# Sreyan88/audio-ssl

Hardware: AMD Instinct MI355X
Metric: upstream clips/sec (1s@16kHz, 64-mel) (higher is better)
Workload: dtype bf16; 1 GPU; delores-m upstream step (log-mel + 2 views + q/k conv encoders + MoCo + 3 Barlow heads + bwd + SGD), 1 s @ 16 kHz, 64 mel, batch 512/GPU, queue 65536; global_batch=512, parallelism=dp1

## Files before the change

### audio-ssl_amd/csrc/conv1.hip

```cpp
#include <cstdlib>
#include "common.h"

namespace {

constexpr int NTAP = 9, NMOM = 9 + 45;
constexpr int MOM_REPL = 16;

__device__ __forceinline__ int tri(int a, int b) {
    return a * 9 - a * (a - 1) / 2 + (b - a);
}

constexpr int MOM_TC = 128;
__global__ __launch_bounds__(256) void conv1_moments_kernel(const float* __restrict__ img, double* __restrict__ mom,
                                                            int N, int F, int T, int nchunk, int tcw) {
    extern __shared__ float tile[];
    __shared__ float sh[4][NMOM];
    const int n = blockIdx.x / nchunk, t0 = (blockIdx.x - n * nchunk) * tcw;
    const int tc = min(tcw, T - t0), ld = tc + 2;
    const float* im = img + (long)n * F * T;
    {
        const int total = (F + 2) * ld, dr = 256 / ld, dc = 256 - dr * ld;
        int r = threadIdx.x / ld, cidx = threadIdx.x - r * ld;
        for (int i0 = threadIdx.x; i0 < total; i0 += 8 * 256) {
            float v[8];
            int rr = r, cc = cidx;
#pragma unroll
            for (int k = 0; k < 8; ++k) {
                const int f = rr - 1, t = t0 + cc - 1;
                v[k] = (i0 + k * 256 < total && f >= 0 && f < F && t >= 0 && t < T) ? im[f * T + t] : 0.f;
                cc += dc; rr += dr;
                if (cc >= ld) { cc -= ld; ++rr; }
            }
#pragma unroll
            for (int k = 0; k < 8; ++k)
                if (i0 + k * 256 < total) tile[i0 + k * 256] = v[k];
            r = rr; cidx = cc;
        }
    }
    __syncthreads();
    float acc[NMOM];
#pragma unroll
    for (int i = 0; i < NMOM; ++i) acc[i] = 0.f;
    const int df = 256 / tc, dt = 256 - df * tc;
    int f = threadIdx.x / tc, t = threadIdx.x - f * tc;
    for (; f < F;) {
        const float* c = tile + f * ld + t;
        float x[NTAP];
#pragma unroll
        for (int kh = 0; kh < 3; ++kh)
#pragma unroll
            for (int kw = 0; kw < 3; ++kw) x[kh * 3 + kw] = c[kh * ld + kw];
#pragma unroll
        for (int a = 0; a < 9; ++a) {
            acc[a] += x[a];
#pragma unroll
            for (int b = 0; b < 9; ++b)
                if (b >= a) acc[9 + tri(a, b)] += x[a] * x[b];
        }
        t += dt; f += df;
        if (t >= tc) { t -= tc; ++f; }
    }
    const int lane = threadIdx.x & 63, w = threadIdx.x >> 6;
#pragma unroll
    for (int i = 0; i < NMOM; ++i) {
        const float v = wave_sum(acc[i]);
        if (lane == 0) sh[w][i] = v;
    }
    __syncthreads();
    if (threadIdx.x < NMOM) {
        const double v = (double)sh[0][threadIdx.x] + (double)sh[1][threadIdx.x] + (double)sh[2][threadIdx.x] +
                         (double)sh[3][threadIdx.x];
        atomicAdd(&mom[(blockIdx.x & (MOM_REPL - 1)) * NMOM + threadIdx.x], v);
    }
}

__global__ __launch_bounds__(576) void conv1_finalize_kernel(double* __restrict__ momr, const float* __restrict__ w,
                                      const float* __restrict__ bias, const float* __restrict__ gamma,
                                      const float* __restrict__ beta, float* running_mean, float* running_var,
                                      float momentum, float eps, double count, float* scale, float* shift,
                                      float* save_mean, float* save_rstd, int repl) {
    __shared__ double tot[NMOM];
    __shared__ double cov[81];
    __shared__ double rowv[64][9], rowm[64][9];
    const int i = threadIdx.x;
    if (i < NMOM) {
        double t = 0.0;
        for (int r = 0; r < repl; ++r) t += momr[r * NMOM + i];
        tot[i] = t;
    }
    __syncthreads();
    if (i < NMOM) momr[i] = tot[i];
    if (i < 81) {
        const int a = i / 9, bb = i - a * 9;
        const double s2 = tot[9 + (a <= bb ? tri(a, bb) : tri(bb, a))] / count;
        cov[i] = s2 - (tot[a] / count) * (tot[bb] / count);
    }
    __syncthreads();
    const int c = i / 9, a = i - (i / 9) * 9;
    if (i < 576) {
        double r = 0.0;
        for (int bb = 0; bb < 9; ++bb) r += (double)w[c * 9 + bb] * cov[a * 9 + bb];
        rowv[c][a] = (double)w[c * 9 + a] * r;
        rowm[c][a] = (double)w[c * 9 + a] * tot[a];
    }
    __syncthreads();
    if (i < 576 && a == 0) {
        double mean = 0.0, var = 0.0;
        for (int k = 0; k < 9; ++k) { mean += rowm[c][k]; var += rowv[c][k]; }
        mean = mean / count;
        var = var < 0.0 ? 0.0 : var;
        mean += (double)bias[c];
        const double rstd = 1.0 / sqrt(var + (double)eps);
        const float sc = (float)((double)gamma[c] * rstd);
        scale[c] = sc;
        shift[c] = (float)((double)beta[c] - mean * (double)gamma[c] * rstd);
        save_mean[c] = (float)mean;
        save_rstd[c] = (float)rstd;
        if (running_mean) {
            running_mean[c] = (1.f - momentum) * running_mean[c] + momentum * (float)mean;
            running_var[c] = (1.f - momentum) * running_var[c] + momentum * (float)(var * count / (count - 1.0));
        }
    }
}

__device__ __forceinline__ void load_patch(float* patch, const float* __restrict__ img, int n, int tp, int F, int T) {
    const float* im = img + (long)n * F * T;
    for (int i = threadIdx.x; i < (F + 2) * 4; i += 256) {
        const int f = (i >> 2) - 1, t = 2 * tp - 1 + (i & 3);
        patch[i] = (f >= 0 && f < F && t >= 0 && t < T) ? im[f * T + t] : 0.f;
    }
}

struct PatchRegs {
    float v[2];
    __device__ __forceinline__ void fetch(const float* __restrict__ img, int n, int tp, int F, int T) {
        const float* im = img + (long)n * F * T;
#pragma unroll
        for (int j = 0; j < 2; ++j) {
            const int i = threadIdx.x + j * 256;
            const int f = (i >> 2) - 1, t = 2 * tp - 1 + (i & 3);
            v[j] = (i < (F + 2) * 4 && f >= 0 && f < F && t >= 0 && t < T) ? im[f * T + t] : 0.f;
        }
    }
    __device__ __forceinline__ void put(float* patch, int F) const {
#pragma unroll
// ... 135 lines not shown
__device__ __forceinline__ Vec8<bf16> stem_taps(const float* patch, int f, int dt, int half) {
    Vec8<bf16> a;
    if (half == 0) {
        a.v[0] = (bf16)patch[(f + 0) * 4 + dt + 0]; a.v[1] = (bf16)patch[(f + 0) * 4 + dt + 1]; a.v[2] = (bf16)patch[(f + 0) * 4 + dt + 2];
        a.v[3] = (bf16)patch[(f + 1) * 4 + dt + 0]; a.v[4] = (bf16)patch[(f + 1) * 4 + dt + 1]; a.v[5] = (bf16)patch[(f + 1) * 4 + dt + 2];
        a.v[6] = (bf16)patch[(f + 2) * 4 + dt + 0]; a.v[7] = (bf16)patch[(f + 2) * 4 + dt + 1];
    } else {
        a = Vec8<bf16>::zero();
        a.v[0] = (bf16)patch[(f + 2) * 4 + dt + 2];
    }
    return a;
}
__device__ __forceinline__ Vec8<bf16> stem_weights(const float* w, int c, int half) {
    Vec8<bf16> b = Vec8<bf16>::zero();
    if (half == 0) {
#pragma unroll
        for (int jj = 0; jj < 8; ++jj) b.v[jj] = (bf16)w[c * 9 + jj];
    } else {
        b.v[0] = (bf16)w[c * 9 + 8];
    }
    return b;
}

__global__ __launch_bounds__(256) void conv1_fwd_mfma_kernel(const float* __restrict__ img, const float* __restrict__ w,
                                                             const float* __restrict__ bias, const float* __restrict__ scale,
                                                             const float* __restrict__ shift, bf16* __restrict__ out,
                                                             float* __restrict__ xl, int XS, int N, int F, int T) {
    extern __shared__ __attribute__((aligned(16))) float patch[];
    const int lane = threadIdx.x & 63, wv = threadIdx.x >> 6, half = lane >> 5, l31 = lane & 31;
    const int To = T / 2, Fo = F / 2;
    bf16* const stage = reinterpret_cast<bf16*>(patch + (((F + 2) * 4 + 3) & ~3));
    Vec8<bf16> wb[2];
    float b[2], sc[2], sh[2];
#pragma unroll
    for (int j = 0; j < 2; ++j) {
        const int c = 32 * j + l31;
        wb[j] = stem_weights(w, c, half);
        b[j] = bias[c]; sc[j] = scale[c]; sh[j] = shift[c];
    }
    const int pp = l31 >> 2, df = (l31 >> 1) & 1, dt = l31 & 1;
    PatchRegs pre;
    int item, step, end;
    if (xl) {
        const int n = blockIdx.x / XS, s4 = blockIdx.x - n * XS, per = (To + XS - 1) / XS;
        item = n * To + s4 * per; step = 1; end = n * To + min(To, (s4 + 1) * per);
    } else {
        item = blockIdx.x; step = gridDim.x; end = N * To;
    }
    float xs[2][2][4];
#pragma unroll
    for (int u = 0; u < 2; ++u)
#pragma unroll
        for (int j = 0; j < 2; ++j)
#pragma unroll
            for (int q = 0; q < 4; ++q) xs[u][j][q] = 0.f;
    if (item < end) { pre.fetch(img, item / To, item % To, F, T); pre.put(patch, F); }
    __syncthreads();
    for (; item < end; item += step) {
        const int n = item / To, tp = item - n * To;
        const int nxt = item + step;
        if (nxt < end) pre.fetch(img, nxt / To, nxt % To, F, T);
// ... 213 lines not shown
    }
    __syncthreads();
    if (lstat) {
        if (i < 64) { lstat[i] = (float)s11[i * 11 + 9]; lstat[64 + i] = (float)s11[i * 11 + 10]; }
        return;
    }
    if (i < 576) {
        const int c = i / 9, t = i - c * 9;
        const double db = gstat ? (double)gstat[c] : s11[c * 11 + 9], dg = gstat ? (double)gstat[64 + c] : s11[c * 11 + 10];
        const double rs = rstd[c], mu = mean[c], gm = gamma[c];
        double wS2 = 0.0;
        for (int a = 0; a < 9; ++a) wS2 += (double)w[c * 9 + a] * mom[9 + (a <= t ? tri(a, t) : tri(t, a))];
        const double yhat_x = rs * (wS2 + ((double)bias[c] - mu) * mom[t]);
        const double v = gm * rs * (s11[c * 11 + t] - db / count * mom[t] - dg / count * yhat_x);
        dW[c * 9 + t] += (float)v;
    }
    if (i < 64) {
        dgamma[i] += (float)s11[i * 11 + 10];
        dbeta[i] += (float)s11[i * 11 + 9];
    }
    (void)dbias;
}

void launch_moments(const float* img, double* mom, int N, int F, int T, hipStream_t s) {
    const int tcw = MOM_TC;
    const int nchunk = ceil_div(T, tcw);
    const size_t lds = sizeof(float) * (F + 2) * (min(T, tcw) + 2);
    hipLaunchKernelGGL(conv1_moments_kernel, dim3(N * nchunk), dim3(256), lds, s, img, mom, N, F, T, nchunk, tcw);
}

}

extern "C" int audiossl_conv1_stats(const float* img, int N, int F, int T, const float* w, const float* bias,
                                    const float* gamma, const float* beta, float* running_mean, float* running_var,
                                    float momentum, float eps, double* mom, float* scale, float* shift,
                                    float* save_mean, float* save_rstd, void* stream) {
    ASSL_REQUIRE(img && w && bias && gamma && beta && mom && scale && shift && save_mean && save_rstd);
    ASSL_REQUIRE(N > 0 && F >= 2 && F <= 120 && T >= 2 && (long)N * F * T < 0x7FFFFFFFL - 0x1000000L);
    hipStream_t s = static_cast<hipStream_t>(stream);
    ASSL_ZERO(mom, sizeof(double) * NMOM * MOM_REPL, s);
    const long total = (long)N * F * T;
    launch_moments(img, mom, N, F, T, s);
    hipLaunchKernelGGL(conv1_finalize_kernel, dim3(1), dim3(576), 0, s, mom, w, bias, gamma, beta, running_mean,
                       running_var, momentum, eps, (double)total, scale, shift, save_mean, save_rstd, MOM_REPL);
    ASSL_LAUNCH_CHECK();
}

__global__ void conv1_fold_kernel(double* __restrict__ momr) {
    __shared__ double tot[NMOM];
    const int c = threadIdx.x;
    if (c < NMOM) {
        double t = 0.0;
        for (int r = 0; r < MOM_REPL; ++r) t += momr[r * NMOM + c];
        tot[c] = t;
    }
    __syncthreads();
    if (c < NMOM) momr[c] = tot[c];
}
extern "C" int audiossl_conv1_moments(const float* img, int N, int F, int T, double* mom, void* stream) {
    ASSL_REQUIRE(img && mom && N > 0 && F >= 2 && F <= 120 && T >= 2 && (long)N * F * T < 0x7FFFFFFFL - 0x1000000L);
    hipStream_t s = static_cast<hipStream_t>(stream);
    ASSL_ZERO(mom, sizeof(double) * NMOM * MOM_REPL, s);
    launch_moments(img, mom, N, F, T, s);
    hipLaunchKernelGGL(conv1_fold_kernel, dim3(1), dim3(64), 0, s, mom);
    ASSL_LAUNCH_CHECK();
}
extern "C" int audiossl_conv1_finalize(double* mom_totals, const float* w, const float* bias, const float* gamma, const float* beta,
                                       float* running_mean, float* running_var, float momentum, float eps, double count,
                                       float* scale, float* shift, float* save_mean, float* save_rstd, void* stream) {
    ASSL_REQUIRE(mom_totals && w && bias && gamma && beta && scale && shift && save_mean && save_rstd && count > 1.0);
    hipLaunchKernelGGL(conv1_finalize_kernel, dim3(1), dim3(576), 0, static_cast<hipStream_t>(stream), mom_totals, w, bias, gamma, beta,
                       running_mean, running_var, momentum, eps, count, scale, shift, save_mean, save_rstd, 1);
    ASSL_LAUNCH_CHECK();
}

extern "C" int audiossl_conv1_fwd(int dtype, const float* img, int N, int F, int T, const float* w, const float* bias,
                                  const float* scale, const float* shift, void* out, float* xl, void* stream) {
    ASSL_REQUIRE(img && w && bias && scale && shift && out && N > 0 && F >= 2 && F <= 126 && T >= 2 && (F % 2) == 0);
    ASSL_REQUIRE(dtype == 0 || dtype == 1 || dtype == 2);
    ASSL_REQUIRE(!xl || dtype == 1);
    hipStream_t s = static_cast<hipStream_t>(stream);
    const int xs_split = 4;
    const int grid = xl ? N * xs_split : min(N * (T / 2), 2048);
    size_t lds = sizeof(float) * (F + 2) * 4;
    if (dtype == 1) lds = sizeof(float) * (((F + 2) * 4 + 3) & ~3) + sizeof(bf16) * (F / 2) * 64;
    if (dtype == 0)
        hipLaunchKernelGGL(conv1_fwd_kernel<float>, dim3(grid), dim3(256), lds, s, img, w, bias, scale, shift,
                           static_cast<float*>(out), N, F, T);
    else if (dtype == 2)
        hipLaunchKernelGGL(conv1_fwd_kernel<bf16>, dim3(grid), dim3(256), lds, s, img, w, bias, scale, shift,
                           static_cast<bf16*>(out), N, F, T);
    else
        hipLaunchKernelGGL(conv1_fwd_mfma_kernel, dim3(grid), dim3(256), lds, s, img, w, bias, scale, shift,
                           static_cast<bf16*>(out), xl, xs_split, N, F, T);
    ASSL_LAUNCH_CHECK();
}

static int conv1_bwd_main(int dtype, int conv_dtype, const float* img, int N, int F, int T, const float* w, const float* bias,
                                  const float* gamma, const float* scale, const float* shift, const float* mean,
                                  const float* rstd, const double* mom, const void* dP, const void* dxl, float* acc,
                                  void* stream) {
    ASSL_REQUIRE(img && w && bias && gamma && scale && shift && mean && rstd && mom && dP && acc);
    ASSL_REQUIRE(N > 0 && F >= 2 && F <= 64 && T >= 2 && (F % 2) == 0 && (dtype == 0 || dtype == 1));
    hipStream_t s = static_cast<hipStream_t>(stream);
    ASSL_ZERO(acc, sizeof(float) * 32 * 64 * 11, s);
    static const int bwd_grid = getenv("AUDIOSSL_CONV1_BWD_GRID") ? atoi(getenv("AUDIOSSL_CONV1_BWD_GRID")) : 2048;
    const int grid = min(N * (T / 2), bwd_grid);
    const size_t lds = sizeof(float) * (F + 2) * 4;
    const float inv_To = 1.f / (float)(T / 2);
    if (conv_dtype == 1 && F == 64 && dtype == 0)
        hipLaunchKernelGGL((conv1_bwd_mfma_kernel<true, float>), dim3(grid), dim3(256), lds + 2 * 2048 * sizeof(float), s, img, w, bias, scale,
                           shift, mean, rstd, static_cast<const float*>(dP), static_cast<const float*>(dxl), inv_To, acc, N, F, T);
    else if (conv_dtype == 1 && F == 64)
        hipLaunchKernelGGL((conv1_bwd_mfma_kernel<true, bf16>), dim3(grid), dim3(256), lds + 2 * 2048 * sizeof(float), s, img, w, bias, scale,
                           shift, mean, rstd, static_cast<const bf16*>(dP), static_cast<const float*>(dxl), inv_To, acc, N, F, T);
    else if (conv_dtype == 1 && dtype == 0)
        hipLaunchKernelGGL((conv1_bwd_mfma_kernel<false, float>), dim3(grid), dim3(256), lds, s, img, w, bias, scale, shift, mean, rstd,
// ... 45 lines not shown
```

### audio-ssl_amd/src/engine.py

```python
import os

import torch

from src import _native as N

import os as _os
_STEM_VALU = _os.environ.get("AUDIOSSL_STEM_VALU") == "1"
BN_MOMENTUM = 0.1
BN_EPS = 1e-5
_BN_FUSED = _os.environ.get("AUDIOSSL_BN_FUSED", "1") != "0"


ONE_STREAM = os.environ.get("AUDIOSSL_ONE_STREAM", "0") == "1"


_CAPTURE_ORIGIN = []


class capture_scope:

    def __enter__(self):
        _CAPTURE_ORIGIN.append(torch.cuda.current_stream())
        return self

# ... 270 lines not shown
        return Y, Pout, (st[0], st[1], st[2], st[3]), Wf, Wd
    if train and fused:
        st = _empty((4, 64), torch.float32, like=Pin)
        sq = sq[0]
        SYNC_BN.all_reduce(sq)
        N.call("bn_finalize", sq[0], sq[1], 1, float(M * SYNC_BN.world), 64, gamma, beta, rm if update_running else None,
               rv if update_running else None, BN_MOMENTUM, BN_EPS, st[0], st[1], st[2], st[3])
        scale, shift, mean, rstd = st[0], st[1], st[2], st[3]
    elif train:
        scale, shift, mean, rstd = _bn_train(ad, Y, M, 64, gamma, beta, rm, rv, update_running)
    else:
        scale, shift = _bn_eval(Y, 64, gamma, beta, rm, rv)
        mean = rstd = None
    N.call("bn_relu_pool_fwd", dtype, ad, Y, scale, shift, Pout, Nimg, Ti, Fi)
    return Y, Pout, (scale, shift, mean, rstd), Wf, Wd


def _col_buffer(dtype, Nimg, T1, F1, like):
    if dtype == N.BF16 and F1 in (16, 32):
        return None
    return _empty((Nimg * T1 * F1, 576), N.torch_dtype(dtype), like=like)


def encoder_forward(P, x, dtype, keep=None, p_drop=0.3, train=True, update_running=True, want_layers=True, Wc=None,
                    layer_out=None, before_fc=None):
    Nimg, _, F, T = x.shape
    assert F == 64, "the HIP encoder is built for n_mels = 64 (the reference's only setting)"
    td = N.torch_dtype(dtype)
    c = EncoderCtx()
    c.P = P
    c.dtype, c.N, c.F, c.T, c.train, c.p_drop = dtype, Nimg, F, T, train, p_drop
    img = x.reshape(Nimg, F, T).contiguous()
    c.img = img
    w1 = P["features_1.0.weight"].reshape(64, 9)
    b1 = P["features_1.0.bias"]
    g1, be1 = P["features_1.1.weight"], P["features_1.1.bias"]
    if train:
        c.mom1 = ARENA.scratch((16 * 54,), torch.float64, x)
        c.sc1, c.sh1, c.mean1, c.rstd1 = (_empty((64,), torch.float32, like=x) for _ in range(4))
        rm1 = P["features_1.1.running_mean"] if update_running else None
        rv1 = P["features_1.1.running_var"] if update_running else None
        if SYNC_BN is None:
            N.call("conv1_stats", img, Nimg, F, T, w1, b1, g1, be1, rm1, rv1, BN_MOMENTUM, BN_EPS, c.mom1, c.sc1, c.sh1, c.mean1, c.rstd1)
        else:
            N.call("conv1_moments", img, Nimg, F, T, c.mom1)
            mom_g = SYNC_BN.all_reduce(c.mom1[:54].clone())
            N.call("conv1_finalize", mom_g, w1, b1, g1, be1, rm1, rv1, BN_MOMENTUM, BN_EPS, float(Nimg * F * T * SYNC_BN.world),
                   c.sc1, c.sh1, c.mean1, c.rstd1)
    else:
        c.sc1, c.sh1 = _bn_eval(x, 64, g1, be1, P["features_1.1.running_mean"], P["features_1.1.running_var"])
    T1, F1 = T // 2, F // 2
    c.P1 = _empty((Nimg, T1, F1, 64), td, like=x)
    c.stem_mfma = dtype == N.BF16 and not HP and not _STEM_VALU
    x1 = x2 = x3 = None
    if want_layers:
        x1, x2, x3 = layer_out if layer_out is not None else (_empty((Nimg, f * 64), td, like=x) for f in (F // 2, F // 4, F // 8))
    x1_fused = c.stem_mfma and x1 is not None and x1.dtype == torch.float32 and x1.is_contiguous()
    x1_parts = _empty((4, Nimg, (F // 2) * 64), torch.float32, like=x) if x1_fused else None
    N.call("conv1_fwd", dtype if (dtype == N.F32 or c.stem_mfma) else 2, img, Nimg, F, T, w1, b1, c.sc1, c.sh1, c.P1, x1_parts)
    col = _col_buffer(dtype, Nimg, T1, F1, x)
    bn2 = (P["features_2.1.weight"], P["features_2.1.bias"], P["features_2.1.running_mean"], P["features_2.1.running_var"])
    packs = [_empty((64, 576), td, like=x) for _ in range(4)]
    N.call("pack_conv_w2", dtype, P["features_2.0.weight"], packs[0], packs[1], P["features_3.0.weight"], packs[2], packs[3])
    c.Y2, c.P2, c.st2, c.W2f, c.W2d = _conv_block_fwd(dtype, c.P1, Nimg, T1, F1, P["features_2.0.weight"],
                                                       P["features_2.0.bias"], bn2, train, update_running, col, packed=packs[:2])
    T2, F2 = T1 // 2, F1 // 2
    bn3 = (P["features_3.1.weight"], P["features_3.1.bias"], P["features_3.1.running_mean"], P["features_3.1.running_var"])
    c.Y3, c.P3, c.st3, c.W3f, c.W3d = _conv_block_fwd(dtype, c.P2, Nimg, T2, F2, P["features_3.0.weight"],
                                                       P["features_3.0.bias"], bn3, train, update_running, col, packed=packs[2:])
    del col
    T3, F3 = T2 // 2, F2 // 2
    c.dims = (T1, F1, T2, F2, T3, F3)
    if want_layers:
        o32 = int(x1.dtype == torch.float32)
        N.call("tmean3_fwd", dtype, o32, None if x1_fused else c.P1, x1, x1_parts, T1, F1, c.P2, x2, T2, F2, c.P3, x3, T3, F3, Nimg)
    d = P["fc.0.weight"].shape[0]
    kin = F3 * 64
    M = Nimg * T3
    c.d, c.kin, c.M = d, kin, M
    if before_fc is not None:
        before_fc()
    if Wc is not None:
# ... 448 lines not shown
```

### audio-ssl_amd/src/upstream/delores_m/upstream_expert.py

```python
import os

import torch
import torch.nn as nn

from src import _native as N
from src import engine as E
from src.encoder.audiontt import default_precision
from src.flat import FlatGroup
from src.module_base import UpstreamModule
from src.upstream.common import EAGER, FusedExpertMixin, FusedStepFn, MocoQueueMixin, Projection, strip
from src.upstream.delores_m.upstream_encoder import DELORES_M as DELORES_M_ENCODER
from src.utils import concat_all_gather


_PREP_ASIDE = os.environ.get("AUDIOSSL_PREP_ASIDE", "1") != "0"
_HEADS_ASIDE = os.environ.get("AUDIOSSL_HEADS_ASIDE", "1") != "0"
_FUSED_SGD = os.environ.get("AUDIOSSL_FUSED_SGD", "1") != "0"
_SKIP_ZERO = os.environ.get("AUDIOSSL_SKIP_ZERO", "1") != "0"
_GRADS_ZERO = os.environ.get("AUDIOSSL_GRADS_ZERO", "1") != "0"
_DY_EVENT = os.environ.get("AUDIOSSL_DY_EVENT", "1") != "0"
_LATE_JOIN = os.environ.get("AUDIOSSL_LATE_JOIN", "1") != "0"
_SGD_ASIDE = os.environ.get("AUDIOSSL_SGD_ASIDE", "1") != "0"


def _world():
    import torch.distributed as dist
    return dist.get_world_size() if dist.is_available() and dist.is_initialized() else 1


class Upstream_Expert(MocoQueueMixin, FusedExpertMixin, UpstreamModule):
    prefer_phases = False

    def __init__(self, config, base_encoder, datamodule=None, emb_dim: int = 128, num_negatives: int = 65536,
                 encoder_momentum: float = 0.999, softmax_temperature: float = 0.07, learning_rate: float = 0.03,
                 momentum: float = 0.9, weight_decay: float = 1e-4, data_dir: str = './', batch_size: int = 256,
                 use_mlp: bool = False, num_workers: int = 8, *args, **kwargs):
        super().__init__()
        self.save_hyperparameters()
        if use_mlp:
            raise NotImplementedError("use_mlp is not part of the HIP path")
        self.config = config
        self.base_encoder = base_encoder
        self.datamodule = datamodule
        self.encoder_q, self.encoder_k = self.init_encoders(self.base_encoder)
        for param_q, param_k in zip(self.encoder_q.parameters(), self.encoder_k.parameters()):
# ... 22 lines not shown
        named += [(n, p) for n, p in self.named_parameters() if n.startswith(("p1.", "p2.", "p3."))]
        return named

    def fused_loss(self, img_q, img_k, need_grad=True, parts=None, runner=None, optimizer=None):
        with E.ARENA.step(img_q.device):
            return self._fused_loss(img_q, img_k, need_grad, parts, runner, optimizer)

    def _fused_loss(self, img_q, img_k, need_grad, parts, runner, optimizer):
        R = runner or EAGER
        dt = self.precision
        E.set_high_precision(self.high_precision)
        flat = self.ensure_flat()
        dev = img_q.device
        B = img_q.shape[0]
        eq, ek = self.encoder_q, self.encoder_k
        ddp = _world() > 1
        img_k = img_k.float().contiguous()
        img_q = img_q.float().contiguous()
        pending_k = self._shuffle_begin(img_k) if ddp else None
        main = torch.cuda.current_stream()
        G = flat.grad_dict
        Ys = R.alloc("Ys", lambda: [torch.empty(2 * B, f, dtype=E.pooled_dtype(dt), device=dev) for f in (2048, 1024, 512)])

        def key_phase(x):
            self._momentum_update_key_encoder(shadow_dtype=dt)
            self.flat_k.refresh_shadow(dt)
            Wk = self.flat_k.shadow_dict()
            keepk = ek.encoder.next_keep_mask(B, x.shape[-1])
            _, _, _, Hk, _ = E.encoder_forward(ek.encoder.param_dict(), x, dt, keep=keepk, p_drop=0.3, train=self.training,
                                               Wc=strip(Wk, "encoder."), layer_out=tuple(y[B:] for y in Ys))
            yk, _ = E.maxmean_forward(dt, Hk)
            wk = Wk["fc.weight"]
            return E.linear_fwd(dt, yk, wk, B, wk.shape[0], wk.shape[1], bias=ek.fc.bias.data, out_f32=1)

        def key_branch():
            x, idx_unshuffle = img_k, None
            if ddp:
                x, idx_unshuffle = self._shuffle_end(pending_k, B)
                x = R.static("key_in", x)
            kk = R.phase("key", lambda: key_phase(x))
            if ddp:
                kk = R.static("key_out", self._batch_unshuffle_ddp(kk, idx_unshuffle))
            return kk
        k = self._key_stream.run(dev, key_branch)

        heads = (self.p1, self.p2, self.p3)
        grouped = not (self.high_precision or dt == N.F32 or not self.grouped_heads or E.SYNC_BN is not None)
        D_ = self.p1.param_dict()["projector.3.weight"].shape[0]
        kins_ = [p.param_dict()["projector.0.weight"].shape[1] for p in heads]
        stored_grads = tuple(f"p{i + 1}.projector.{j}.weight" for i in range(3) for j in (0, 3, 6)) \
            if (need_grad and grouped and _GRADS_ZERO and _SKIP_ZERO and E.heads_wgrads_store(D_, kins_, 2 * B)) else ()

        sgd_ctx = None
        if stored_grads and _FUSED_SGD and optimizer is not None and not ddp and hasattr(optimizer, "fused_wgrad"):
            sgd_ctx = optimizer.fused_wgrad(flat, [f"p{i + 1}." for i in range(3)])

        def query_phase():
            def prep():
                if need_grad:
                    flat.zero_grad(stores_ok=bool(stored_grads))
                flat.refresh_shadow(dt)
            busy = (need_grad and not (flat._fresh_grad is True or (flat._fresh_grad == "partial" and stored_grads))) or \
                   not (flat._fresh_shadow or dt == N.F32)
            if _PREP_ASIDE and busy:
                self._prep_stream.run(dev, prep)
            else:
                prep()
            Wq = flat.shadow_dict("encoder_q.")
            wq = Wq["fc.weight"]
            fold = not (self.high_precision or dt == N.F32 or not self.grouped_heads)
            loss = torch.zeros(4 + (3 * E.LOSS_REPLICAS if fold else 0), dtype=torch.float32, device=dev)
            keep = eq.encoder.next_keep_mask(B, img_q.shape[-1])
            _, _, _, Hq, cq = E.encoder_forward(eq.encoder.param_dict(), img_q, dt, keep=keep, p_drop=0.3, train=self.training,
                                                Wc=strip(Wq, "encoder."), layer_out=tuple(y[:B] for y in Ys),
                                                before_fc=(lambda: self._prep_stream.join(dev)) if (_PREP_ASIDE and busy) else None)
            yq, argq = E.maxmean_forward(dt, Hq)
            q = E.linear_fwd(dt, yq, wq, B, wq.shape[0], wq.shape[1], bias=eq.fc.bias.data, out_f32=1)
            return loss, wq, Hq, cq, yq, argq, q
        loss, wq, Hq, cq, yq, argq, q = R.phase("query", query_phase)
        self._key_stream.join(dev)
        k.record_stream(main)

        streams = self._streams(dev)
        dys = [None, None, None]
        dy_event = None

        def head_phase(i, p):
            Wp = flat.shadow_dict(f"p{i + 1}.")
            return E.barlow_forward_backward(p.param_dict(), G(f"p{i + 1}."), Ys[i], dt, p.lambd, p.scale_loss,
                                             loss[i + 1:i + 2], need_dy1=True, need_dy2=False,
                                             update_running=self.training, backward=need_grad,
                                             Wc=tuple(Wp[f"projector.{j}.weight"] for j in (0, 3, 6)))
        if not grouped:
            for i, p in enumerate(heads):
                if not E.ONE_STREAM:
                    E.fork(streams[i], main)
                with torch.cuda.stream(streams[i]):
                    dys[i] = R.phase(f"head{i + 1}", lambda i=i, p=p: head_phase(i, p))
# ... 108 lines not shown
```

### include/audiossl_hip.h

```cpp
#ifndef AUDIOSSL_HIP_H
#define AUDIOSSL_HIP_H

#include <stdint.h>

#ifdef __cplusplus
extern "C" {
#endif

#define AUDIOSSL_OK 0
#define AUDIOSSL_EINVAL (-1)
#define AUDIOSSL_ELAUNCH (-2)
#define AUDIOSSL_EALIGN (-3)

int audiossl_logmel_fwd(const float* wave, float* out, int B, int L, int T, int n_fft, int hop, int n_mels, int taps,
                        const float* win, const float* tw, const float* melw, const int* mel_start, float eps_pow,
                        float eps_log, int apply_log, void* stream);

int audiossl_fbank_fwd(const float* wave, const int* lens, const int* partner, const float* lam, float* clip_mean,
                       const int* bands, const int* bands_host, float* out, int B, int Lmax, int win_len, int shift, int n_fft, int n_mels,
                       int taps, int T_target, const float* win, const float* tw, const float* melw, const int* mel_start,
                       float preemph, float eps_log, float mean, float std, int skip_norm, int time_major, void* stream);

int audiossl_clip_moments(const float* x, double* mom, int B, int n, void* stream);
int audiossl_runnorm_scan(const double* mom, int B, int n_elem, long long* state_i, float* state_f, float* mu_out,
// ... 7 lines not shown
                           int use_rrc, double fs_lo, double fs_hi, double ts_lo, double ts_hi, int canvas_h,
                           int canvas_w, int use_spec, int spec_F, int spec_T, int spec_nf, int spec_nt, const int* lens,
                           int unit, int* starts, int* ip, float* fp, int* masks);

int audiossl_resample_sinc(const float* x, float* y, int clips, int n_orig, int n_out, const int* n, const int* off_l,
                           const int* off_r, const double* eta_l, const double* eta_r, const double* win, const double* delta,
                           int nwin, int index_step, void* stream);

int audiossl_pcm_window(const void* pcm, long pcm_bytes, const long long* tab, const long long* tab_host, float* out, int B,
                        int unit, int align, void* stream);

int audiossl_kmix_cluster(const float* views, const float* centroids, int n_views, int F, int T, int K, int* cluster,
                          void* stream);
int audiossl_kmix_apply(const float* views, const float* ring, const int* slot, const float* coef, int n_views, int n,
                        int log_mix, float* out, void* stream);
int audiossl_mask_fill(float* x, const int* tab, int n_img, int max_masks, int F, int T, int zero_fill, void* stream);

int audiossl_conv1_stats(const float* img, int N, int F, int T, const float* w, const float* bias, const float* gamma,
                         const float* beta, float* running_mean, float* running_var, float momentum, float eps,
                         double* mom, float* scale, float* shift, float* save_mean, float* save_rstd, void* stream);
#define AUDIOSSL_CONV1_XL_PARTS 4
int audiossl_conv1_fwd(int dtype, const float* img, int N, int F, int T, const float* w, const float* bias,
                       const float* scale, const float* shift, void* out, float* xl, void* stream);
int audiossl_conv1_bwd(int dtype, int conv_dtype, const float* img, int N, int F, int T, const float* w, const float* bias,
                       const float* gamma, const float* scale, const float* shift, const float* mean, const float* rstd,
                       const double* mom, const void* dP, const void* dxl, float* acc, float* dW, float* dbias,
                       float* dgamma, float* dbeta, void* stream);

int audiossl_colstats(int dtype, const void* x, int groups, long M, int C, long ld, int want_sq, double* sum,
                      double* sumsq, void* stream);
int audiossl_bn_finalize(const double* sum, const double* sumsq, int groups, double count, int C, const float* gamma,
                         const float* beta, float* running_mean, float* running_var, float momentum, float eps,
                         float* scale, float* shift, float* save_mean, float* save_rstd, void* stream);
int audiossl_bn_relu_pool_fwd(int dtype, int ydtype, const void* Y, const float* scale, const float* shift, void* P, int N,
                              int Ti, int Fi, void* stream);
int audiossl_bn_relu_pool_train_fwd(int dtype, int ydtype, const void* Y, const double* sum, const double* sumsq, int stat_replicas,
                                    double count, const float* gamma, const float* beta, float* running_mean, float* running_var,
                                    float momentum, float eps, void* P, float* scale, float* shift, float* save_mean, float* save_rstd,
                                    int N, int Ti, int Fi, void* stream);
int audiossl_tmean_fwd(int dtype, int out_f32, const void* P, void* xl, int N, int To, int Fo, void* stream);
int audiossl_tmean3_fwd(int dtype, int out_f32, const void* P1, void* x1, const float* x1_parts, int To1, int Fo1, const void* P2,
                        void* x2, int To2, int Fo2, const void* P3, void* x3, int To3, int Fo3, int N, void* stream);
int audiossl_bn_relu_pool_bwd(int dtype, int ydtype, int gdtype, const void* Y, const void* dP, const void* dxl, const float* scale,
                              const float* shift, const float* mean, const float* rstd, float* stat, void* dY,
                              float* dgamma, float* dbeta, int N, int Ti, int Fi, void* stream);
int audiossl_bn_relu_pool_bwd_p(int dtype, int ydtype, int gdtype, const void* Y, const void* P, const void* dP, const void* dxl,
// ... 182 lines not shown
```

Measured before the change: 274,200 clips/s.

## Fuse stem BN finalize into conv1 forward and rework moments kernel

The stem moments kernel is rewritten as a persistent grid over band/chunk tiles with register prefetch of the next tile, packed f32x2 FMA accumulation, and a transpose-style wave reduction. The separate single-block BN finalize launch is folded into a templated training variant of the conv1 MFMA forward kernel, where every block recomputes scale/shift from the moment replicas and block 0 publishes the stats. An optional env-gated path computes q and k view moments in one launch. This removes a tiny serial finalize kernel and improves moment throughput, at the cost of redundant per-block finalize work in every conv1 forward block.

```diff
diff --git a/audio-ssl_amd/csrc/conv1.hip b/audio-ssl_amd/csrc/conv1.hip
--- a/audio-ssl_amd/csrc/conv1.hip
+++ b/audio-ssl_amd/csrc/conv1.hip
@@ -3,124 +3,202 @@
 
 namespace {
 
-constexpr int NTAP = 9, NMOM = 9 + 45;
+constexpr int NMOM = 9 + 45;
 constexpr int MOM_REPL = 16;
 
 __device__ __forceinline__ int tri(int a, int b) {
     return a * 9 - a * (a - 1) / 2 + (b - a);
 }
 
-constexpr int MOM_TC = 128;
-__global__ __launch_bounds__(256) void conv1_moments_kernel(const float* __restrict__ img, double* __restrict__ mom,
-                                                            int N, int F, int T, int nchunk, int tcw) {
-    extern __shared__ float tile[];
-    __shared__ float sh[4][NMOM];
-    const int n = blockIdx.x / nchunk, t0 = (blockIdx.x - n * nchunk) * tcw;
-    const int tc = min(tcw, T - t0), ld = tc + 2;
-    const float* im = img + (long)n * F * T;
-    {
-        const int total = (F + 2) * ld, dr = 256 / ld, dc = 256 - dr * ld;
-        int r = threadIdx.x / ld, cidx = threadIdx.x - r * ld;
-        for (int i0 = threadIdx.x; i0 < total; i0 += 8 * 256) {
-            float v[8];
-            int rr = r, cc = cidx;
-#pragma unroll
-            for (int k = 0; k < 8; ++k) {
-                const int f = rr - 1, t = t0 + cc - 1;
-                v[k] = (i0 + k * 256 < total && f >= 0 && f < F && t >= 0 && t < T) ? im[f * T + t] : 0.f;
-                cc += dc; rr += dr;
-                if (cc >= ld) { cc -= ld; ++rr; }
+constexpr int MOM_SLOT = (1 + MOM_REPL) * NMOM;
+
+constexpr int MOM_BAND = 16, MOM_TC = 128;
+constexpr int MOM_TILE = (MOM_BAND + 2) * (MOM_TC + 2);
+constexpr int MOM_PRE = (MOM_TILE + 255) / 256;
+constexpr int MOM_RUN = 32;
+
+typedef __attribute__((ext_vector_type(2))) float f32x2;
+constexpr int MOM_NPK = 29;
+__device__ __forceinline__ constexpr int mom_pk(int a, int j) {
+    int base = 0;
+    for (int r = 0; r < a; ++r) base += 5 - r / 2;
+    return base + (j - a / 2);
+}
+
+struct MomItem { const float* im; int f0, rows, t0, tc; };
+__device__ __forceinline__ MomItem mom_item(const float* __restrict__ img, int item, int F, int T, int nband, int nchunk) {
+    const int per = nband * nchunk, n = item / per, rem = item - n * per, b = rem / nchunk, ch = rem - b * nchunk;
+    MomItem it;
+    it.im = img + (long)n * F * T;
+    it.f0 = b * MOM_BAND; it.rows = min(MOM_BAND, F - it.f0);
+    it.t0 = ch * MOM_TC;  it.tc = min(MOM_TC, T - it.t0);
+    return it;
+}
+struct MomRegs {
+    float v[MOM_PRE];
+    __device__ __forceinline__ void fetch(const MomItem& it, int F, int T) {
+        const int ld = it.tc + 2, total = (it.rows + 2) * ld;
+        const float inv = 1.f / (float)ld;
+#pragma unroll
+        for (int k = 0; k < MOM_PRE; ++k) {
+            const int i = threadIdx.x + k * 256;
+            const int r = (int)(((float)i + 0.5f) * inv), f = it.f0 - 1 + r, t = it.t0 - 1 + (i - r * ld);
+            v[k] = (i < total && f >= 0 && f < F && t >= 0 && t < T) ? it.im[f * T + t] : 0.f;
+        }
+    }
+    __device__ __forceinline__ void put(float* tile, const MomItem& it) const {
+        const int total = (it.rows + 2) * (it.tc + 2);
+#pragma unroll
+        for (int k = 0; k < MOM_PRE; ++k) {
+            const int i = threadIdx.x + k * 256;
+            if (i < total) tile[i] = v[k];
+        }
+    }
+};
+
+template <int H>
+__device__ __forceinline__ void wave_transpose_sum(float (&v)[64], int lane) {
+    const bool up = (lane & H) != 0;
+#pragma unroll
+    for (int k = 0; k < H; ++k) {
+        const float send = up ? v[k] : v[k + H], keep = up ? v[k + H] : v[k];
+        v[k] = keep + __shfl_xor(send, H, 64);
+    }
+    if constexpr (H > 1) wave_transpose_sum<H / 2>(v, lane);
+}
+
+__global__ __launch_bounds__(256, 4) void conv1_moments_kernel(const float* __restrict__ img_a, const float* __restrict__ img_b,
+                                                               double* __restrict__ rep_a, double* __restrict__ rep_b,
+                                                               int N, int F, int T, int nband, int nchunk) {
+    __shared__ float tile[MOM_TILE];
+    __shared__ float sh[4][64];
+    const float* __restrict__ img = blockIdx.y ? img_b : img_a;
+    double* __restrict__ rep = blockIdx.y ? rep_b : rep_a;
+    const int items = N * nband * nchunk;
+    f32x2 acc2[MOM_NPK];
+#pragma unroll
+    for (int i = 0; i < MOM_NPK; ++i) acc2[i] = f32x2{0.f, 0.f};
+    MomRegs pre;
+    MomItem cur = {}, nx = {};
+    int item = blockIdx.x;
+    if (item < items) { cur = mom_item(img, item, F, T, nband, nchunk); pre.fetch(cur, F, T); }
+    while (item < items) {
+        pre.put(tile, cur);
+        __syncthreads();
+        const int nxt = item + gridDim.x;
+        if (nxt < items) { nx = mom_item(img, nxt, F, T, nband, nchunk); pre.fetch(nx, F, T); }
+        const int ld = cur.tc + 2, npix = cur.rows * cur.tc;
+        const float inv = 1.f / (float)cur.tc;
+        for (int p = threadIdx.x; p < npix; p += 256) {
+            const int f = (int)(((float)p + 0.5f) * inv), t = p - f * cur.tc;
+            const float* c = tile + f * ld + t;
+            float x[10];
+#pragma unroll
+            for (int kh = 0; kh < 3; ++kh)
+#pragma unroll
+                for (int kw = 0; kw < 3; ++kw) x[kh * 3 + kw] = c[kh * ld + kw];
+            x[9] = 1.f;
+#pragma unroll
+            for (int a = 0; a < 9; ++a) {
+                const f32x2 xa = {x[a], x[a]};
+#pragma unroll
+                for (int j = a / 2; j < 5; ++j)
+                    acc2[mom_pk(a, j)] = __builtin_elementwise_fma(xa, f32x2{x[2 * j], x[2 * j + 1]}, acc2[mom_pk(a, j)]);
             }
-#pragma unroll
-            for (int k = 0; k < 8; ++k)
-                if (i0 + k * 256 < total) tile[i0 + k * 256] = v[k];
-            r = rr; cidx = cc;
-        }
-    }
-    __syncthreads();
-    float acc[NMOM];
-#pragma unroll
-    for (int i = 0; i < NMOM; ++i) acc[i] = 0.f;
-    const int df = 256 / tc, dt = 256 - df * tc;
-    int f = threadIdx.x / tc, t = threadIdx.x - f * tc;
-    for (; f < F;) {
-        const float* c = tile + f * ld + t;
-        float x[NTAP];
-#pragma unroll
-        for (int kh = 0; kh < 3; ++kh)
-#pragma unroll
-            for (int kw = 0; kw < 3; ++kw) x[kh * 3 + kw] = c[kh * ld + kw];
-#pragma unroll
-        for (int a = 0; a < 9; ++a) {
-            acc[a] += x[a];
-#pragma unroll
-            for (int b = 0; b < 9; ++b)
-                if (b >= a) acc[9 + tri(a, b)] += x[a] * x[b];
-        }
-        t += dt; f += df;
-        if (t >= tc) { t -= tc; ++f; }
+        }
+        __syncthreads();
+        item = nxt; cur = nx;
+    }
+    float acc[64];
+#pragma unroll
+    for (int i = 0; i < 64; ++i) acc[i] = 0.f;
+#pragma unroll
+    for (int a = 0; a < 9; ++a) {
+        acc[a] = acc2[mom_pk(a, 4)][1];
+#pragma unroll
+        for (int b = a; b < 9; ++b) acc[9 + tri(a, b)] = acc2[mom_pk(a, b / 2)][b & 1];
     }
     const int lane = threadIdx.x & 63, w = threadIdx.x >> 6;
-#pragma unroll
-    for (int i = 0; i < NMOM; ++i) {
-        const float v = wave_sum(acc[i]);
-        if (lane == 0) sh[w][i] = v;
-    }
+    wave_transpose_sum<32>(acc, lane);
+    sh[w][lane] = acc[0];
     __syncthreads();
     if (threadIdx.x < NMOM) {
         const double v = (double)sh[0][threadIdx.x] + (double)sh[1][threadIdx.x] + (double)sh[2][threadIdx.x] +
                          (double)sh[3][threadIdx.x];
-        atomicAdd(&mom[(blockIdx.x & (MOM_REPL - 1)) * NMOM + threadIdx.x], v);
-    }
-}
-
-__global__ __launch_bounds__(576) void conv1_finalize_kernel(double* __restrict__ momr, const float* __restrict__ w,
-                                      const float* __restrict__ bias, const float* __restrict__ gamma,
-                                      const float* __restrict__ beta, float* running_mean, float* running_var,
-                                      float momentum, float eps, double count, float* scale, float* shift,
-                                      float* save_mean, float* save_rstd, int repl) {
-    __shared__ double tot[NMOM];
-    __shared__ double cov[81];
-    __shared__ double rowv[64][9], rowm[64][9];
-    const int i = threadIdx.x;
-    if (i < NMOM) {
+        atomicAdd(&rep[(blockIdx.x & (MOM_REPL - 1)) * NMOM + threadIdx.x], v);
+    }
+}
+
+struct StemBnLds {
+    double tot[NMOM], cov[81], rowv[64 * 9];
+    float sc[64], sh[64];
+};
+struct StemBn {
+    double* slot;
+    const float *gamma, *beta;
+    float *running_mean, *running_var;
+    float momentum, eps;
+    double count;
+    float *scale, *shift, *save_mean, *save_rstd;
+};
+template <int NT>
+__device__ __forceinline__ void stem_bn_finalize(StemBnLds& L, const double* rep, int repl, double* tot_out,
+                                                 const float* __restrict__ w, const float* __restrict__ bias, const StemBn& bn,
+                                                 bool publish) {
+    const double count = bn.count;
+    for (int i = threadIdx.x; i < NMOM; i += NT) {
         double t = 0.0;
-        for (int r = 0; r < repl; ++r) t += momr[r * NMOM + i];
-        tot[i] = t;
-    }
-    __syncthreads();
-    if (i < NMOM) momr[i] = tot[i];
-    if (i < 81) {
+        for (int r = 0; r < repl; ++r) t += rep[r * NMOM + i];
+        L.tot[i] = t;
+    }
+    __syncthreads();
+    if (tot_out)
+        for (int i = threadIdx.x; i < NMOM; i += NT) tot_out[i] = L.tot[i];
+    for (int i = threadIdx.x; i < 81; i += NT) {
         const int a = i / 9, bb = i - a * 9;
-        const double s2 = tot[9 + (a <= bb ? tri(a, bb) : tri(bb, a))] / count;
-        cov[i] = s2 - (tot[a] / count) * (tot[bb] / count);
-    }
-    __syncthreads();
-    const int c = i / 9, a = i - (i / 9) * 9;
-    if (i < 576) {
+        const double s2 = L.tot[9 + (a <= bb ? tri(a, bb) : tri(bb, a))] / count;
+        L.cov[i] = s2 - (L.tot[a] / count) * (L.tot[bb] / count);
+    }
+    __syncthreads();
+    for (int i = threadIdx.x; i < 576; i += NT) {
+        const int c = i / 9, a = i - c * 9;
         double r = 0.0;
-        for (int bb = 0; bb < 9; ++bb) r += (double)w[c * 9 + bb] * cov[a * 9 + bb];
-        rowv[c][a] = (double)w[c * 9 + a] * r;
-        rowm[c][a] = (double)w[c * 9 + a] * tot[a];
-    }
-    __syncthreads();
-    if (i < 576 && a == 0) {
+        for (int bb = 0; bb < 9; ++bb) r += (double)w[c * 9 + bb] * L.cov[a * 9 + bb];
+        L.rowv[i] = (double)w[c * 9 + a] * r;
+    }
+    __syncthreads();
+    for (int c = threadIdx.x; c < 64; c += NT) {
         double mean = 0.0, var = 0.0;
-        for (int k = 0; k < 9; ++k) { mean += rowm[c][k]; var += rowv[c][k]; }
+        {
+#pragma clang fp contract(off)
+            for (int k = 0; k < 9; ++k) { mean += (double)w[c * 9 + k] * L.tot[k]; var += L.rowv[c * 9 + k]; }
+        }
         mean = mean / count;
         var = var < 0.0 ? 0.0 : var;
         mean += (double)bias[c];
-        const double rstd = 1.0 / sqrt(var + (double)eps);
-        const float sc = (float)((double)gamma[c] * rstd);
-        scale[c] = sc;
-        shift[c] = (float)((double)beta[c] - mean * (double)gamma[c] * rstd);
-        save_mean[c] = (float)mean;
-        save_rstd[c] = (float)rstd;
-        if (running_mean) {
-            running_mean[c] = (1.f - momentum) * running_mean[c] + momentum * (float)mean;
-            running_var[c] = (1.f - momentum) * running_var[c] + momentum * (float)(var * count / (count - 1.0));
-        }
-    }
+        const double rstd = 1.0 / sqrt(var + (double)bn.eps);
+        const float sc = (float)((double)bn.gamma[c] * rstd);
+        const float sh = (float)((double)bn.beta[c] - mean * (double)bn.gamma[c] * rstd);
+        L.sc[c] = sc;
+        L.sh[c] = sh;
+        if (publish) {
+            bn.scale[c] = sc;
+            bn.shift[c] = sh;
+            bn.save_mean[c] = (float)mean;
+            bn.save_rstd[c] = (float)rstd;
+            if (bn.running_mean) {
+                bn.running_mean[c] = (1.f - bn.momentum) * bn.running_mean[c] + bn.momentum * (float)mean;
+                bn.running_var[c] = (1.f - bn.momentum) * bn.running_var[c] + bn.momentum * (float)(var * count / (count - 1.0));
+            }
+        }
+    }
+    __syncthreads();
+}
+
+__global__ __launch_bounds__(576) void conv1_finalize_kernel(double* __restrict__ momr, const float* __restrict__ w,
+                                                             const float* __restrict__ bias, StemBn bn, int repl) {
+    __shared__ StemBnLds L;
+    stem_bn_finalize<576>(L, momr, repl, momr, w, bias, bn, true);
 }
 
 __device__ __forceinline__ void load_patch(float* patch, const float* __restrict__ img, int n, int tp, int F, int T) {
@@ -302,21 +380,30 @@
     return b;
 }
 
+template <bool TRAIN>
 __global__ __launch_bounds__(256) void conv1_fwd_mfma_kernel(const float* __restrict__ img, const float* __restrict__ w,
                                                              const float* __restrict__ bias, const float* __restrict__ scale,
                                                              const float* __restrict__ shift, bf16* __restrict__ out,
-                                                             float* __restrict__ xl, int XS, int N, int F, int T) {
+                                                             float* __restrict__ xl, int XS, int N, int F, int T, StemBn bn) {
     extern __shared__ __attribute__((aligned(16))) float patch[];
     const int lane = threadIdx.x & 63, wv = threadIdx.x >> 6, half = lane >> 5, l31 = lane & 31;
     const int To = T / 2, Fo = F / 2;
     bf16* const stage = reinterpret_cast<bf16*>(patch + (((F + 2) * 4 + 3) & ~3));
     Vec8<bf16> wb[2];
     float b[2], sc[2], sh[2];
+    if (TRAIN) {
+        StemBnLds& L = *reinterpret_cast<StemBnLds*>(patch);
+        stem_bn_finalize<256>(L, bn.slot + NMOM, MOM_REPL, blockIdx.x == 0 ? bn.slot : nullptr, w, bias, bn, blockIdx.x == 0);
+#pragma unroll
+        for (int j = 0; j < 2; ++j) { sc[j] = L.sc[32 * j + l31]; sh[j] = L.sh[32 * j + l31]; }
+        __syncthreads();
+    }
 #pragma unroll
     for (int j = 0; j < 2; ++j) {
         const int c = 32 * j + l31;
         wb[j] = stem_weights(w, c, half);
-        b[j] = bias[c]; sc[j] = scale[c]; sh[j] = shift[c];
+        b[j] = bias[c];
+        if (!TRAIN) { sc[j] = scale[c]; sh[j] = shift[c]; }
     }
     const int pp = l31 >> 2, df = (l31 >> 1) & 1, dt = l31 & 1;
     PatchRegs pre;
@@ -576,11 +663,16 @@
     (void)dbias;
 }
 
-void launch_moments(const float* img, double* mom, int N, int F, int T, hipStream_t s) {
-    const int tcw = MOM_TC;
-    const int nchunk = ceil_div(T, tcw);
-    const size_t lds = sizeof(float) * (F + 2) * (min(T, tcw) + 2);
-    hipLaunchKernelGGL(conv1_moments_kernel, dim3(N * nchunk), dim3(256), lds, s, img, mom, N, F, T, nchunk, tcw);
+int launch_moments(const float* img_a, const float* img_b, double* rep_a, double* rep_b, int N, int F, int T, hipStream_t s) {
+    const int nband = ceil_div(F, MOM_BAND), nchunk = ceil_div(T, MOM_TC), items = N * nband * nchunk, views = img_b ? 2 : 1;
+    static const int resident = getenv("AUDIOSSL_MOM_GRID") ? atoi(getenv("AUDIOSSL_MOM_GRID")) : 1024;
+    const int grid = min(items, max(max(resident / views, 1), ceil_div(items, MOM_RUN)));
+    hipLaunchKernelGGL(conv1_moments_kernel, dim3(grid, views), dim3(256), 0, s, img_a, img_b, rep_a, rep_b, N, F, T, nband, nchunk);
+    return hipGetLastError() == hipSuccess ? ASSL_OK : ASSL_ELAUNCH;
+}
+
+bool moments_shape_ok(int N, int F, int T) {
+    return N > 0 && F >= 2 && F <= 120 && T >= 2 && (long)N * F * T < 0x7FFFFFFFL - 0x1000000L;
 }
 
 }
@@ -590,14 +682,21 @@
                                     float momentum, float eps, double* mom, float* scale, float* shift,
                                     float* save_mean, float* save_rstd, void* stream) {
     ASSL_REQUIRE(img && w && bias && gamma && beta && mom && scale && shift && save_mean && save_rstd);
-    ASSL_REQUIRE(N > 0 && F >= 2 && F <= 120 && T >= 2 && (long)N * F * T < 0x7FFFFFFFL - 0x1000000L);
+    ASSL_REQUIRE(moments_shape_ok(N, F, T));
     hipStream_t s = static_cast<hipStream_t>(stream);
     ASSL_ZERO(mom, sizeof(double) * NMOM * MOM_REPL, s);
-    const long total = (long)N * F * T;
-    launch_moments(img, mom, N, F, T, s);
-    hipLaunchKernelGGL(conv1_finalize_kernel, dim3(1), dim3(576), 0, s, mom, w, bias, gamma, beta, running_mean,
-                       running_var, momentum, eps, (double)total, scale, shift, save_mean, save_rstd, MOM_REPL);
+    if (launch_moments(img, nullptr, mom, nullptr, N, F, T, s) != ASSL_OK) return ASSL_ELAUNCH;
+    const StemBn bn = {nullptr, gamma, beta, running_mean, running_var, momentum, eps, (double)((long)N * F * T),
+                       scale, shift, save_mean, save_rstd};
+    hipLaunchKernelGGL(conv1_finalize_kernel, dim3(1), dim3(576), 0, s, mom, w, bias, bn, MOM_REPL);
     ASSL_LAUNCH_CHECK();
+}
+
+extern "C" int audiossl_conv1_moments_pair(const float* img_a, const float* img_b, int N, int F, int T, double* mom, void* stream) {
+    ASSL_REQUIRE(img_a && mom && moments_shape_ok(N, F, T));
+    hipStream_t s = static_cast<hipStream_t>(stream);
+    ASSL_ZERO(mom, sizeof(double) * MOM_SLOT * (img_b ? 2 : 1), s);
+    return launch_moments(img_a, img_b, mom + NMOM, mom + MOM_SLOT + NMOM, N, F, T, s);
 }
 
 __global__ void conv1_fold_kernel(double* __restrict__ momr) {
@@ -612,10 +711,10 @@
     if (c < NMOM) momr[c] = tot[c];
 }
 extern "C" int audiossl_conv1_moments(const float* img, int N, int F, int T, double* mom, void* stream) {
-    ASSL_REQUIRE(img && mom && N > 0 && F >= 2 && F <= 120 && T >= 2 && (long)N * F * T < 0x7FFFFFFFL - 0x1000000L);
+    ASSL_REQUIRE(img && mom && moments_shape_ok(N, F, T));
     hipStream_t s = static_cast<hipStream_t>(stream);
     ASSL_ZERO(mom, sizeof(double) * NMOM * MOM_REPL, s);
-    launch_moments(img, mom, N, F, T, s);
+    if (launch_moments(img, nullptr, mom, nullptr, N, F, T, s) != ASSL_OK) return ASSL_ELAUNCH;
     hipLaunchKernelGGL(conv1_fold_kernel, dim3(1), dim3(64), 0, s, mom);
     ASSL_LAUNCH_CHECK();
 }
@@ -623,8 +722,8 @@
                                        float* running_mean, float* running_var, float momentum, float eps, double count,
                                        float* scale, float* shift, float* save_mean, float* save_rstd, void* stream) {
     ASSL_REQUIRE(mom_totals && w && bias && gamma && beta && scale && shift && save_mean && save_rstd && count > 1.0);
-    hipLaunchKernelGGL(conv1_finalize_kernel, dim3(1), dim3(576), 0, static_cast<hipStream_t>(stream), mom_totals, w, bias, gamma, beta,
-                       running_mean, running_var, momentum, eps, count, scale, shift, save_mean, save_rstd, 1);
+    const StemBn bn = {nullptr, gamma, beta, running_mean, running_var, momentum, eps, count, scale, shift, save_mean, save_rstd};
+    hipLaunchKernelGGL(conv1_finalize_kernel, dim3(1), dim3(576), 0, static_cast<hipStream_t>(stream), mom_totals, w, bias, bn, 1);
     ASSL_LAUNCH_CHECK();
 }
 
@@ -645,8 +744,24 @@
         hipLaunchKernelGGL(conv1_fwd_kernel<bf16>, dim3(grid), dim3(256), lds, s, img, w, bias, scale, shift,
                            static_cast<bf16*>(out), N, F, T);
     else
-        hipLaunchKernelGGL(conv1_fwd_mfma_kernel, dim3(grid), dim3(256), lds, s, img, w, bias, scale, shift,
-                           static_cast<bf16*>(out), xl, xs_split, N, F, T);
+        hipLaunchKernelGGL(conv1_fwd_mfma_kernel<false>, dim3(grid), dim3(256), lds, s, img, w, bias, scale, shift,
+                           static_cast<bf16*>(out), xl, xs_split, N, F, T, StemBn{});
+    ASSL_LAUNCH_CHECK();
+}
+
+extern "C" int audiossl_conv1_fwd_train(const float* img, int N, int F, int T, double* mom, double count, const float* w,
+                                        const float* bias, const float* gamma, const float* beta, float* running_mean,
+                                        float* running_var, float momentum, float eps, float* scale, float* shift,
+                                        float* save_mean, float* save_rstd, void* out, float* xl, void* stream) {
+    ASSL_REQUIRE(img && mom && w && bias && gamma && beta && scale && shift && save_mean && save_rstd && out && count > 1.0);
+    ASSL_REQUIRE(N > 0 && F >= 2 && F <= 126 && T >= 2 && (F % 2) == 0 && (!running_mean == !running_var));
+    hipStream_t s = static_cast<hipStream_t>(stream);
+    const int xs_split = 4;
+    const int grid = xl ? N * xs_split : min(N * (T / 2), 2048);
+    const size_t lds = max(sizeof(float) * (((F + 2) * 4 + 3) & ~3) + sizeof(bf16) * (F / 2) * 64, sizeof(StemBnLds));
+    const StemBn bn = {mom, gamma, beta, running_mean, running_var, momentum, eps, count, scale, shift, save_mean, save_rstd};
+    hipLaunchKernelGGL(conv1_fwd_mfma_kernel<true>, dim3(grid), dim3(256), lds, s, img, w, bias, (const float*)nullptr,
+                       (const float*)nullptr, static_cast<bf16*>(out), xl, xs_split, N, F, T, bn);
     ASSL_LAUNCH_CHECK();
 }
 
diff --git a/audio-ssl_amd/src/engine.py b/audio-ssl_amd/src/engine.py
--- a/audio-ssl_amd/src/engine.py
+++ b/audio-ssl_amd/src/engine.py
@@ -316,8 +316,24 @@
     return _empty((Nimg * T1 * F1, 576), N.torch_dtype(dtype), like=like)
 
 
+MOM_SLOT = 17 * 54
+
+
+def stem_fused(dtype, train=True):
+    return bool(train) and dtype == N.BF16 and not HP and not _STEM_VALU and SYNC_BN is None
+
+
+def stem_moments_pair(xa, xb=None):
+    Nimg, _, F, T = xa.shape
+    assert xb is None or xb.shape == xa.shape
+    mom = ARENA.scratch((1 if xb is None else 2, MOM_SLOT), torch.float64, xa)
+    N.call("conv1_moments_pair", xa.reshape(Nimg, F, T).contiguous(), None if xb is None else xb.reshape(Nimg, F, T).contiguous(),
+           Nimg, F, T, mom)
+    return mom
+
+
 def encoder_forward(P, x, dtype, keep=None, p_drop=0.3, train=True, update_running=True, want_layers=True, Wc=None,
-                    layer_out=None, before_fc=None):
+                    layer_out=None, before_fc=None, stem_moments=None):
     Nimg, _, F, T = x.shape
     assert F == 64, "the HIP encoder is built for n_mels = 64 (the reference's only setting)"
     td = N.torch_dtype(dtype)
@@ -329,11 +345,18 @@
     w1 = P["features_1.0.weight"].reshape(64, 9)
     b1 = P["features_1.0.bias"]
     g1, be1 = P["features_1.1.weight"], P["features_1.1.bias"]
+    c.stem_mfma = dtype == N.BF16 and not HP and not _STEM_VALU
+    fused = stem_fused(dtype, train)
+    assert stem_moments is None or fused, "precomputed stem moments are for the fused bf16 training stem only"
+    rm1 = rv1 = None
     if train:
-        c.mom1 = ARENA.scratch((16 * 54,), torch.float64, x)
         c.sc1, c.sh1, c.mean1, c.rstd1 = (_empty((64,), torch.float32, like=x) for _ in range(4))
         rm1 = P["features_1.1.running_mean"] if update_running else None
         rv1 = P["features_1.1.running_var"] if update_running else None
+    if fused:
+        c.mom1 = stem_moments if stem_moments is not None else stem_moments_pair(x)[0]
+    elif train:
+        c.mom1 = ARENA.scratch((16 * 54,), torch.float64, x)
         if SYNC_BN is None:
             N.call("conv1_stats", img, Nimg, F, T, w1, b1, g1, be1, rm1, rv1, BN_MOMENTUM, BN_EPS, c.mom1, c.sc1, c.sh1, c.mean1, c.rstd1)
         else:
@@ -345,13 +368,16 @@
         c.sc1, c.sh1 = _bn_eval(x, 64, g1, be1, P["features_1.1.running_mean"], P["features_1.1.running_var"])
     T1, F1 = T // 2, F // 2
     c.P1 = _empty((Nimg, T1, F1, 64), td, like=x)
-    c.stem_mfma = dtype == N.BF16 and not HP and not _STEM_VALU
     x1 = x2 = x3 = None
     if want_layers:
         x1, x2, x3 = layer_out if layer_out is not None else (_empty((Nimg, f * 64), td, like=x) for f in (F // 2, F // 4, F // 8))
     x1_fused = c.stem_mfma and x1 is not None and x1.dtype == torch.float32 and x1.is_contiguous()
     x1_parts = _empty((4, Nimg, (F // 2) * 64), torch.float32, like=x) if x1_fused else None
-    N.call("conv1_fwd", dtype if (dtype == N.F32 or c.stem_mfma) else 2, img, Nimg, F, T, w1, b1, c.sc1, c.sh1, c.P1, x1_parts)
+    if fused:
+        N.call("conv1_fwd_train", img, Nimg, F, T, c.mom1, float(Nimg * F * T), w1, b1, g1, be1, rm1, rv1, BN_MOMENTUM, BN_EPS,
+               c.sc1, c.sh1, c.mean1, c.rstd1, c.P1, x1_parts)
+    else:
+        N.call("conv1_fwd", dtype if (dtype == N.F32 or c.stem_mfma) else 2, img, Nimg, F, T, w1, b1, c.sc1, c.sh1, c.P1, x1_parts)
     col = _col_buffer(dtype, Nimg, T1, F1, x)
     bn2 = (P["features_2.1.weight"], P["features_2.1.bias"], P["features_2.1.running_mean"], P["features_2.1.running_var"])
     packs = [_empty((64, 576), td, like=x) for _ in range(4)]
diff --git a/audio-ssl_amd/src/upstream/delores_m/upstream_expert.py b/audio-ssl_amd/src/upstream/delores_m/upstream_expert.py
--- a/audio-ssl_amd/src/upstream/delores_m/upstream_expert.py
+++ b/audio-ssl_amd/src/upstream/delores_m/upstream_expert.py
@@ -21,6 +21,7 @@
 _DY_EVENT = os.environ.get("AUDIOSSL_DY_EVENT", "1") != "0"
 _LATE_JOIN = os.environ.get("AUDIOSSL_LATE_JOIN", "1") != "0"
 _SGD_ASIDE = os.environ.get("AUDIOSSL_SGD_ASIDE", "1") != "0"
+_STEM_PAIR = os.environ.get("AUDIOSSL_STEM_PAIR", "0") == "1"
 
 
 def _world():
@@ -89,13 +90,20 @@
         G = flat.grad_dict
         Ys = R.alloc("Ys", lambda: [torch.empty(2 * B, f, dtype=E.pooled_dtype(dt), device=dev) for f in (2048, 1024, 512)])
 
+        moms = None
+        if _STEM_PAIR and not ddp and E.stem_fused(dt, self.training):
+            moms = R.phase("stem_moments", lambda: E.stem_moments_pair(img_q, img_k))
+            if not E.ONE_STREAM:
+                moms.record_stream(self._key_stream.stream(dev))
+
         def key_phase(x):
             self._momentum_update_key_encoder(shadow_dtype=dt)
             self.flat_k.refresh_shadow(dt)
             Wk = self.flat_k.shadow_dict()
             keepk = ek.encoder.next_keep_mask(B, x.shape[-1])
             _, _, _, Hk, _ = E.encoder_forward(ek.encoder.param_dict(), x, dt, keep=keepk, p_drop=0.3, train=self.training,
-                                               Wc=strip(Wk, "encoder."), layer_out=tuple(y[B:] for y in Ys))
+                                               Wc=strip(Wk, "encoder."), layer_out=tuple(y[B:] for y in Ys),
+                                               stem_moments=None if moms is None else moms[1])
             yk, _ = E.maxmean_forward(dt, Hk)
             wk = Wk["fc.weight"]
             return E.linear_fwd(dt, yk, wk, B, wk.shape[0], wk.shape[1], bias=ek.fc.bias.data, out_f32=1)
@@ -140,7 +148,8 @@
             keep = eq.encoder.next_keep_mask(B, img_q.shape[-1])
             _, _, _, Hq, cq = E.encoder_forward(eq.encoder.param_dict(), img_q, dt, keep=keep, p_drop=0.3, train=self.training,
                                                 Wc=strip(Wq, "encoder."), layer_out=tuple(y[:B] for y in Ys),
-                                                before_fc=(lambda: self._prep_stream.join(dev)) if (_PREP_ASIDE and busy) else None)
+                                                before_fc=(lambda: self._prep_stream.join(dev)) if (_PREP_ASIDE and busy) else None,
+                                                stem_moments=None if moms is None else moms[0])
             yq, argq = E.maxmean_forward(dt, Hq)
             q = E.linear_fwd(dt, yq, wq, B, wq.shape[0], wq.shape[1], bias=eq.fc.bias.data, out_f32=1)
             return loss, wq, Hq, cq, yq, argq, q
diff --git a/include/audiossl_hip.h b/include/audiossl_hip.h
--- a/include/audiossl_hip.h
+++ b/include/audiossl_hip.h
@@ -53,6 +53,12 @@
 #define AUDIOSSL_CONV1_XL_PARTS 4
 int audiossl_conv1_fwd(int dtype, const float* img, int N, int F, int T, const float* w, const float* bias,
                        const float* scale, const float* shift, void* out, float* xl, void* stream);
+#define AUDIOSSL_CONV1_MOM_SLOT (17 * 54)
+int audiossl_conv1_moments_pair(const float* img_a, const float* img_b, int N, int F, int T, double* mom, void* stream);
+int audiossl_conv1_fwd_train(const float* img, int N, int F, int T, double* mom, double count, const float* w, const float* bias,
+                             const float* gamma, const float* beta, float* running_mean, float* running_var, float momentum,
+                             float eps, float* scale, float* shift, float* save_mean, float* save_rstd, void* out, float* xl,
+                             void* stream);
 int audiossl_conv1_bwd(int dtype, int conv_dtype, const float* img, int N, int F, int T, const float* w, const float* bias,
                        const float* gamma, const float* scale, const float* shift, const float* mean, const float* rstd,
                        const double* mom, const void* dP, const void* dxl, float* acc, float* dW, float* dbias,
```

After: 277,300 clips/s, median of 6. 1.01x the previous value.
